# EI-CoreBioinformatics/portcullis

Measured on AMD Instinct MI355X. Metric: junc_reads_per_sec, higher is better.
Workload: dtype int32; 1 GPU; BASELINE configs[2]: synthetic 199999998 paired-end 150-bp reads, 25 contigs of GRCh38 lengths (3088286401 bp), 249999 junctions, orientation FR; reads_total=199999998, junctions_total=249999, contigs=25, reads_rank0=199999998, pairs_rank0=66692850

## Files before the change

### portcullis_amd/csrc/pjb_api.hip

```cpp
#include "pjb_host.hip.h"
#include "pjb_kernels.hip.h"
#include "pjb_chain.hip.h"
#include "pjb_flight.hip.h"

extern "C" {

namespace {
std::mutex g_host_mu;
std::map<void *, size_t> g_host_registered;
}
void *pjb_host_alloc(size_t bytes) {
    if (bytes >= ((size_t)8 << 20)) {
        const size_t huge = (size_t)2 << 20, len = (bytes + huge - 1) & ~(huge - 1);
        void *p = mmap(nullptr, len, PROT_READ | PROT_WRITE, MAP_PRIVATE | MAP_ANONYMOUS, -1, 0);
        if (p != MAP_FAILED) {
            (void)madvise(p, len, MADV_HUGEPAGE);
            const size_t nt = std::min<size_t>(4, len >> 24);
            auto touch = [&](size_t t) {
                const size_t per = ((len / std::max<size_t>(nt, 1)) + huge - 1) & ~(huge - 1), a = std::min(len, per * t), b = std::min(len, a + per);
                for (size_t o = a; o < b; o += 4096) ((volatile uint8_t *)p)[o] = 0;
            };
            if (nt <= 1) touch(0);
            else {
                std::vector<std::thread> th;
// ... 165 lines not shown
    release_pooled_slabs(c);
    if (c->rows_pinned) (void)hipHostFree(c->rows_pinned);
    if (c->rows_table) (void)dev_free(c, c->rows_table);
    bam_stage_clear(c);
    for (int k = 0; k < PJB_MAX_QUEUED; k++) {
        CtlSlot &S = c->sl[k];
        if (S.pub) (void)hipHostFree(S.pub);
        if (S.batches_pinned) (void)hipHostFree(S.batches_pinned);
        for (auto &ev : S.ev)
            if (ev) (void)hipEventDestroy(ev);
        if (S.ev_rows) (void)hipEventDestroy(S.ev_rows);
        if (S.ev_done) (void)hipEventDestroy(S.ev_done);
        Buf *sb[] = {&S.x_q, &S.x_spos, &S.x_send, &S.x_gapoff, &S.x_zlist, &S.x_scnt, &S.x_codes, &S.cstats, &S.err, &S.gencount, &S.batches, &S.rows, &S.tile_cnt, &S.tile_stats, &S.splidx, &S.splpoff, &S.splrec, &S.tile_soff, &S.chunk_tile, &S.scan_parts, &S.members, &S.okey, &S.g,
                     &S.rec, &S.jidbam, &S.jkey, &S.total, &S.bitmap, &S.wrank, &S.pagecnt, &S.pagerank, &S.ends, &S.firstid,
                     &S.key[0], &S.key[1], &S.idx[0], &S.idx[1], &S.hist, &S.hist_scan, &S.hist_part, &S.bintotal, &S.scan_tiles, &S.jid, &S.seg, &S.runfirst,
                     &S.runstart, &S.ent, &S.entsum, &S.frag, &S.fragj, &S.masks, &S.acc, &S.ancl, &S.ancr, &S.genlist, &S.runs};
        for (Buf *b : sb) release(c, *b);
        hipEvent_t evs[] = {S.ev_k1, S.ev_xk1, S.ev_fork, S.ev_join, S.ev_fork2, S.ev_join2};
        for (hipEvent_t e : evs)
            if (e) (void)hipEventDestroy(e);
        if (S.main) (void)hipStreamDestroy(S.main);
        if (S.side) (void)hipStreamDestroy(S.side);
    }
    if (c->mirror_hdr) (void)hipHostFree(c->mirror_hdr);
    for (int k = 0; k < 2; k++) {
        if (c->stage[k]) (void)hipHostFree(c->stage[k]);
        if (c->stage_ev[k]) (void)hipEventDestroy(c->stage_ev[k]);
    }
    Buf *all[] = {&c->b_cursor, &c->b_scan_tiles, &c->b_hasx, &c->b_xtotal, &c->b_fasta_raw, &c->b_inf_comp, &c->b_inf_out, &c->b_inf_blocks, &c->b_inf_status, &c->b_inf_scratch, &c->b_inf_bitmap,
                  &c->b_bam_seg, &c->b_bam_rec, &c->b_bam_ctl, &c->f_pos, &c->f_cigoff, &c->f_cigar, &c->f_codes,
                  &c->x_pos, &c->x_endx, &c->x_q, &c->x_prefq, &c->x_ce, &c->x_bound, &c->x_de, &c->x_dropped, &c->x_zlist, &c->x_cnt,
// ... 476 lines not shown
}

int pjb_set_option(pjb_ctx *c, const char *name, int64_t value) {
    if (!c || !name) return PJB_ERR_ARG;
    if (c->n_fl) return fail(c, PJB_ERR_STATE, "set_option: target %d is still queued", c->fl[0].tid);
    const std::string n = name;
    if (n == "overlap") c->side_stream = value != 0;
    else if (n == "dense_ids") c->dense_ids = value != 0;
    else if (n == "extra_dense") c->extra_dense_only = value != 0;
    else if (n == "sort_floor") c->sort_floor = (u32)std::max<int64_t>(1, std::min<int64_t>(value, 1 << 30));
    else if (n == "window_skip") c->window_skip = value != 0;
    else if (n == "run_sort") c->run_sort = value != 0;
    else if (n == "run_window") {
        if (value < 0 || value > (int64_t)RUN_W) return fail(c, PJB_ERR_ARG, "set_option: run_window takes 0 (the default, %u) to %u", RUN_W, RUN_W);
        c->run_window = (u32)value;
    } else if (n == "pair_range") {
        int shift = -1;
        for (int k = 0; k <= PAIR_RANGE_SHIFT_MAX; k++)
            if (value == (int64_t)1 << k) shift = k;
        if (shift < 0) return fail(c, PJB_ERR_ARG, "set_option: pair_range takes 1, 2, 4, 8, 16 or 32 slices a range (the default: %d)", 1 << PAIR_RANGE_SHIFT_DEFAULT);
        c->pair_range_shift = shift;
    } else if (n == "grow_batch") {
        if (value < 0 || value > 32768) return fail(c, PJB_ERR_ARG, "set_option: grow_batch takes 0 (the default: what the pool holds) to 32768 trees");
        c->model.grow_batch = (u32)value;
    } else if (n == "knn_chunk") {
        if (value < 0 || value > (1 << 22)) return fail(c, PJB_ERR_ARG, "set_option: knn_chunk takes 0 (the default: sized to fill the chip) to %d base rows", 1 << 22);
        c->model.knn_chunk = (u32)value;
    } else if (n == "mem_limit") {
        if (value < 0) return fail(c, PJB_ERR_ARG, "set_option: mem_limit takes 0 (the default: no limit) or a number of bytes");
        std::lock_guard<std::mutex> lk(c->mem.mu);
// ... 47 lines not shown
```

### portcullis_amd/csrc/pjb_chain.hip.h

```cpp
#pragma once

constexpr unsigned K6_BLOCKS = 128;

static size_t rows_upper_bound(const pjb_ctx *c) {
    size_t n = c->rows_n;
    for (int k = 0; k < c->n_fl; k++)
        if (c->fl[k].queued) n += c->fl[k].lim.junc_limit;
    return n;
}

static void wait_flight(pjb_ctx *c, Flight &f) {
    if (f.queued) (void)hipEventSynchronize(c->sl[f.slot].ev_done);
}

static int rows_table_reserve(pjb_ctx *c, Flight &f, u32 JL) {
    size_t old = rows_upper_bound(c);
    if (old + JL <= c->rows_cap) return PJB_OK;
    for (int k = 0; k < c->n_fl; k++)
        if (c->fl[k].queued && &c->fl[k] != &f) wait_flight(c, c->fl[k]);
    int rc = rows_sync(c);
    if (rc) return rc;
    old = std::min(old, c->rows_cap);
    const size_t ncap = std::max<size_t>((old + JL) * 3 / 2, 1024);
    pjb_junction_row *nd = (pjb_junction_row *)dev_alloc(c, MEM_ROWS, ncap * sizeof(pjb_junction_row));
// ... 2 lines not shown
        HIP_TRY(c, hipMemcpyAsync(nd, c->rows_table, old * sizeof(pjb_junction_row), hipMemcpyDeviceToDevice, c->stream4));
        HIP_TRY(c, hipStreamSynchronize(c->stream4));
    }
    if (c->rows_table) bury(c, c->rows_table);
    c->rows_table = nd;
    c->rows_cap = ncap;
    return PJB_OK;
}

struct Chain {
    pjb_ctx *c;
    Flight &f;
    CtlSlot &S;
    hipStream_t st, service;
    GroupTab GT;
    bool group, fast_codes, any_x, stage_events, xk1, dense_moved, entropy_forked;
    int n_members;
    int32_t ref_len;
    KeyFmt kf;
    u32 PL, JL, SL;
    u32 n_tiles, pair_blocks, range_blocks, slots_lim, n_slices_lim, gen_cap, pack_nn;
    int range_shift;
    size_t n_words;
    int64_t row_base, mirror_base;
    u32 rs_tiles, run_cap, ro_tiles, plan_tiles;
    bool run_route, first_hist_done;
    int sort_bits, n_pass, pass_bits[16], cur;
    RunOut ro;
    u64 *ro_total, *ro_key[2];
    u32 *run_dest, *ro_idx[2];
    u64 *d_err;
    ContigStats *d_cs;
    const u32 *d_P, *d_J, *d_slots;
    MemberStats *d_members;
    u32 *d_member_junc, *d_tile_lo, *d_gen_cnt;
    Pairs pr;
};

struct ChainScope {
    pjb_ctx *c;
    hipStream_t stream = c->stream;
    Buf *scan_tiles = c->scan_tiles;
    int pool = c->cur_pool;
    ~ChainScope() {
        c->stream = stream;
// ... 58 lines not shown
    ch.row_base = ahead ? -1 : (int64_t)c->rows_n;
    ch.mirror_base = ahead ? -1 : (int64_t)c->mirror_rows;
    ch.pair_blocks = std::max<u32>(1, (PL + 255) / 256);
    ch.gen_cap = lim.list_cap ? lim.list_cap : (c->list_cap_forced ? c->list_cap_forced : gen_list_cap(PL));
    ch.pack_nn = (u64)ch.n_tiles * K1_TILE < (1ull << 28) ? 1u : 0u;
    ch.range_shift = c->pair_range_shift;
    ch.slots_lim = frag_slots_limit(JL, PL, ch.range_shift);
    ch.range_blocks = std::max<u32>(1, (frag_ranges(PL, ch.range_shift) + 3) / 4);
    ch.n_slices_lim = (PL + 63) / 64 + 1;
    ch.n_words = ((size_t)std::max(ch.ref_len, 1) + 63) / 64;
    ch.stage_events = c->ktime && c->ktime_only.empty();
    ch.xk1 = c->extra && !c->extra_dense_only && !ch.group && !f.x_k1 && !f.x_pre;
    ch.rs_tiles = std::max<u32>(1, (PL + RS_TILE - 1) / RS_TILE);
    ch.run_route = lim.dense && lim.run_sort;
    ch.run_cap = (u32)std::min<u64>((u64)PL / 8 + 64ull * ch.rs_tiles, 0xfff00000ull);
    ch.ro_tiles = (ch.run_cap + RS_TILE - 1) / RS_TILE;
    if (ch.run_route) {
        ch.ro.cap = ch.run_cap;
        ch.ro.window = c->run_window ? std::min<u32>(c->run_window, RUN_W) : RUN_W;
        ch.ro.tile_bits = std::max(1, bits_of((uint64_t)ch.rs_tiles));
    }
    ch.sort_bits = lim.dense ? std::max(1, bits_of((uint64_t)ch.SL)) + (ch.run_route ? ch.ro.tile_bits : 0) : ch.kf.total_bits;
    ch.plan_tiles = ch.run_route ? ch.ro_tiles : ch.rs_tiles;
    ch.first_hist_done = lim.dense && !ch.run_route;
    ch.n_pass = std::max(1, (ch.sort_bits + c->radix_max_bits - 1) / c->radix_max_bits);
    for (int p = 0; p < ch.n_pass; p++) ch.pass_bits[p] = ch.sort_bits / ch.n_pass + (p < ch.sort_bits % ch.n_pass ? 1 : 0);
    return PJB_OK;
}

static RunOut run_carve(Chain &ch, int &rc) {
    pjb_ctx *c = ch.c;
    CtlSlot &S = ch.S;
    RunOut ro = ch.ro;
    auto al = [](size_t b) { return (b + 255) & ~(size_t)255; };
    const u32 rs_tiles = ch.rs_tiles, run_cap = ch.run_cap;
    const size_t slack = (size_t)run_cap + RS_TILE;
    const size_t at_tf = 256, at_tn = at_tf + al((size_t)rs_tiles * 4), at_key = at_tn + al((size_t)rs_tiles * 4), at_cnt = at_key + al(slack * 8),
                 at_dest = at_cnt + al((size_t)run_cap * 4), at_k0 = at_dest + al((size_t)run_cap * 4), at_k1 = at_k0 + al(slack * 8),
                 at_i0 = at_k1 + al(slack * 8), at_i1 = at_i0 + al(slack * 4), at_end = at_i1 + al(slack * 4);
    if ((rc = ensure(c, S.runs, at_end))) return ro;
    uint8_t *b = (uint8_t *)S.runs.p;
    ro.n_runs = (u32 *)b;
    ch.ro_total = (u64 *)(b + 8);
    ro.tile_first = (u32 *)(b + at_tf);
    ro.tile_n = (u32 *)(b + at_tn);
    ro.key = (u64 *)(b + at_key);
    ro.cnt = (u32 *)(b + at_cnt);
    ch.run_dest = (u32 *)(b + at_dest);
    ch.ro_key[0] = (u64 *)(b + at_k0);
    ch.ro_key[1] = (u64 *)(b + at_k1);
    ch.ro_idx[0] = (u32 *)(b + at_i0);
    ch.ro_idx[1] = (u32 *)(b + at_i1);
    return ro;
}

static int chain_room(Chain &ch) {
    pjb_ctx *c = ch.c;
    Flight &f = ch.f;
    CtlSlot &S = ch.S;
    const std::vector<DevBatch> &batches = f.batches;
    const u32 PL = ch.PL, JL = ch.JL, n_tiles = ch.n_tiles;
    const size_t n_words = ch.n_words, N = (size_t)f.n_reads;
    const u32 plan_tiles = ch.plan_tiles;
    const int dbits = ch.pass_bits[0];
    const bool dense = f.lim.dense;
    int rc;
    if (batches.size() + 2 > S.batches_pinned_cap) {
        if (S.batches_pinned) (void)hipHostFree(S.batches_pinned);
        S.batches_pinned = nullptr;
        S.batches_pinned_cap = 0;
        const size_t cap = std::max<size_t>(batches.size() * 2 + 2, 16);
        HIP_TRY(c, hipHostMalloc((void **)&S.batches_pinned, cap * sizeof(DevBatch), hipHostMallocDefault));
        S.batches_pinned_cap = cap;
    }
    memcpy(S.batches_pinned, batches.data(), batches.size() * sizeof(DevBatch));
    const struct { Buf *b; size_t bytes; bool whole; } once[] = {
        {&S.scan_parts, sizeof(ScanPart) * K1S_BLOCKS, false},
        {&c->b_cursor, sizeof(RowCursor), false},
// ... 36 lines not shown
        {&S.frag, (size_t)ch.slots_lim * F_WORDS * 4},
        {&S.fragj, (size_t)ch.slots_lim * 4},
        {&S.acc, (size_t)JL * F_WORDS * 4 + 16},
        {&S.ancl, (size_t)JL * 4 + 16},
        {&S.ancr, (size_t)JL * 4 + 16},
        {&S.jkey, (size_t)JL * 8 + 16},
        {&S.rows, (size_t)JL * sizeof(pjb_junction_row) + 16},
        {&S.entsum, (size_t)JL * 8 + 16},
        {&S.bitmap, n_words * 8 + 16, dense},
        {&S.wrank, n_words * 4 + 16, dense},
        {&S.pagecnt, ((n_words >> KD_PAGE_SHIFT) + 1) * 4 + 16, dense},
        {&S.pagerank, ((n_words >> KD_PAGE_SHIFT) + 1) * 4 + 16, dense},
        {&S.ends, (size_t)JL * DENSE_ENDS * 4 + 32, dense},
        {&S.firstid, (size_t)JL * 4 + 16, dense},
        {&S.masks, (size_t)ch.n_slices_lim * 8 * 2 + (size_t)ch.n_slices_lim * 4, dense},
        {&S.hist, (size_t)plan_tiles * (1u << dbits) * 4},
        {&S.hist_scan, (size_t)plan_tiles * (1u << dbits) * 4},
        {&S.bintotal, (size_t)4 << dbits},
        {&S.hist_part, (size_t)((plan_tiles + RSP_TILES - 1) / RSP_TILES) * (1u << dbits) * 4},
        {&S.x_q, N + 16, ch.xk1},
        {&S.x_spos, N * 4 + 16, ch.xk1},
        {&S.x_send, N * 4 + 16, ch.xk1},
        {&S.x_zlist, (size_t)X_ZCAP * 8, ch.xk1},
        {&S.x_scnt, X_SCNT_BYTES, ch.xk1},
    };
    for (const auto &r : room)
        if (r.on && (rc = ensure(c, *r.b, r.bytes))) return rc;
    ch.dense_moved = was[0] != S.bitmap.p || was[1] != S.ends.p || was[2] != S.pagecnt.p;
    if (ch.run_route) {
        ch.ro = run_carve(ch, rc);
        if (rc) return rc;
    }
    if ((rc = rows_table_reserve(c, f, JL))) return rc;
    if (!S.pub) {
        HIP_TRY(c, hipHostMalloc((void **)&S.pub, PUB_BYTES, hipHostMallocMapped | hipHostMallocPortable));
        void *dp = nullptr;
        if (hipHostGetDevicePointer(&dp, S.pub, 0) != hipSuccess || !dp) return fail(c, PJB_ERR_HIP, "hipHostGetDevicePointer(control block) failed");
        S.pub_dev = (uint8_t *)dp;
    }
    ch.d_members = (MemberStats *)S.members.p;
    ch.d_member_junc = (u32 *)(ch.d_members + GROUP_MAX);
    ch.d_tile_lo = ch.d_member_junc + GROUP_MAX;
    ch.d_err = (u64 *)S.err.p;
    ch.d_cs = (ContigStats *)S.cstats.p;
    ch.d_P = &ch.d_cs->P;
    ch.d_J = &ch.d_cs->J;
    ch.d_slots = &ch.d_cs->n_slots;
// ... 27 lines not shown
    }
    if (!S.at_rest) {
        HIP_TRY(c, hipMemsetAsync(S.err.p, 0xff, 8, st));
        HIP_TRY(c, hipMemsetAsync(S.gencount.p, 0, GEN_SHARDS * GEN_CNT_STRIDE * 4, st));
        HIP_TRY(c, hipMemsetAsync(ch.d_member_junc, 0, GROUP_MAX * 4, st));
    }
    S.at_rest = false;
    HIP_TRY(c, hipEventRecord(S.ev[0], st));
    if (f.lim.dense) {
        if (!S.dense_at_rest || ch.dense_moved) {
            HIP_TRY(c, hipMemsetAsync(S.bitmap.p, 0, S.bitmap.cap, st));
            HIP_TRY(c, hipMemsetAsync(S.pagecnt.p, 0, S.pagecnt.cap, st));
            HIP_TRY(c, hipMemsetAsync(S.ends.p, 0xff, S.ends.cap, st));
        }
        S.dense_at_rest = false;
    }
    f.pr = ch.pr;
    return PJB_OK;
}

static int chain_k1(Chain &ch) {
    pjb_ctx *c = ch.c;
    Flight &f = ch.f;
    CtlSlot &S = ch.S;
    const std::vector<DevBatch> &batches = f.batches;
    const hipStream_t st = ch.st;
    const GroupTab &GT = ch.GT;
    const KeyFmt kf = ch.kf;
    const u32 n_tiles = ch.n_tiles;
    const bool k1_late = getenv("PJB_K1_SERIAL_LATE") != nullptr;
// ... 91 lines not shown
        return rc;
    LAUNCH(c, "kd_table", kd_table, dim3(cand_blocks), dim3(256), (const u64 *)cand, (const u64 *)S.ent.p, (const u32 *)cand_rank, kf, JL,
           (const u32 *)S.ends.p, (const u32 *)S.firstid.p, (const u64 *)S.total.p, (u64 *)S.jkey.p, (int32_t *)S.ancl.p, (int32_t *)S.ancr.p, ch.d_cs,
           (const u32 *)ch.d_gen_cnt, ch.gen_cap, ch.SL, ch.ro.n_runs, ch.range_shift);
    LAUNCH(c, "kd_assign", kd_assign, dim3(ch.rs_tiles), dim3(256), okey, ch.d_P, kf, (const u64 *)S.bitmap.p, (const u32 *)S.wrank.p,
           (const u32 *)S.ends.p, (const u32 *)S.firstid.p, JL, (const u64 *)S.total.p, (u32 *)S.jidbam.p, (u32 *)S.acc.p, (const u64 *)S.jkey.p,
           (const int32_t *)S.ancl.p, (const int32_t *)S.ancr.p, ch.d_err, ch.d_cs, ch.run_route ? 0 : ch.pass_bits[0], (u32 *)S.hist.p, ch.ro);
    if ((rc = chain_fork(ch, S.ev_fork, S.ev_join, f.forked, chain_k4b))) return rc;
    LAUNCH(c, "kd_reset", kd_reset, dim3(cand_blocks), dim3(256), (const u64 *)cand, (const u32 *)cand_rank, kf, JL, (const ContigStats *)ch.d_cs,
           (u64 *)S.bitmap.p, (u32 *)S.ends.p, (u32 *)S.pagecnt.p);
    S.dense_at_rest = true;
    return PJB_OK;
}

static const char *const rs_names[4] = {"rs_hist", "rs_panel_sums", "rs_panel_scan", "rs_scatter"};
static const char *const ro_names[6] = {"ro_hist", "ro_panel_sums", "ro_panel_scan", "ro_scatter", "ro_offsets", "rs_place"};

template <typename K>
static int sort_pass(Chain &ch, const void *kin_v, void *kout_v, const u32 *vin, u32 *vout, int shift, int bits, const u32 *d_n, u32 tiles,
                     const char *const *names) {
    pjb_ctx *c = ch.c;
    CtlSlot &S = ch.S;
    const K *kin = (const K *)kin_v;
    K *kout = (K *)kout_v;
    if (!(shift == 0 && ch.first_hist_done))
        LAUNCH(c, names[0], rs_hist<K>, dim3(tiles), dim3(256), kin, d_n, shift, bits, (u32 *)S.hist.p, tiles);
    {
        const u32 nb = 1u << bits, n_panels = (tiles + RSP_TILES - 1) / RSP_TILES;
        LAUNCH(c, names[1], rs_panel_sums, dim3(n_panels, (nb + 255) / 256), dim3(256), (const u32 *)S.hist.p, tiles, nb, (u32 *)S.hist_part.p);
        LAUNCH(c, names[2], rs_panel_scan, dim3(n_panels, (nb + 255) / 256), dim3(256), (const u32 *)S.hist.p, (const u32 *)S.hist_part.p, tiles, nb,
               (u32 *)S.hist_scan.p, (u32 *)S.bintotal.p);
// ... 5 lines not shown
    case 9: RS_SCATTER(9); break;
    case 10: RS_SCATTER(10); break;
    case 11: RS_SCATTER(11); break;
    default: RS_SCATTER(0); break;
    }
#undef RS_SCATTER
    return PJB_OK;
}

static int chain_sort(Chain &ch) {
    pjb_ctx *c = ch.c;
    Flight &f = ch.f;
    CtlSlot &S = ch.S;
    const RunOut &ro = ch.ro;
    int rc = PJB_OK, cur = 0, shift = 0;
    for (int p = 0; p < ch.n_pass; p++) {
        const int bits = ch.pass_bits[p];
        if (bits <= 0) break;
        if (ch.run_route) {
            rc = sort_pass<u64>(ch, p == 0 ? (const void *)ro.key : (const void *)ch.ro_key[cur], ch.ro_key[cur ^ 1], p == 0 ? nullptr : (const u32 *)ch.ro_idx[cur],
                                ch.ro_idx[cur ^ 1], shift, bits, (const u32 *)ro.n_runs, ch.ro_tiles, ro_names);
        } else {
            const u32 *vin = p == 0 ? nullptr : (const u32 *)S.idx[cur].p;
            u32 *vout = (u32 *)S.idx[cur ^ 1].p;
            if (f.lim.dense) rc = sort_pass<u32>(ch, p == 0 ? S.jidbam.p : S.key[cur].p, S.key[cur ^ 1].p, vin, vout, shift, bits, ch.d_P, ch.rs_tiles, rs_names);
            else rc = sort_pass<u64>(ch, p == 0 ? S.okey.p : S.key[cur].p, S.key[cur ^ 1].p, vin, vout, shift, bits, ch.d_P, ch.rs_tiles, rs_names);
        }
        if (rc) return rc;
        cur ^= 1;
        shift += bits;
    }
    f.n_pass = ch.n_pass;
    if (ch.run_route) {
        const u32 *order = ch.ro_idx[cur];
        if ((rc = run_scan(c, ro_names[4], RunCountFn{(const u32 *)ro.cnt, order}, RunDestSink{ch.run_dest, order}, (u64)ch.run_cap, ch.ro_total, (const u32 *)ro.n_runs)))
            return rc;
        cur = 1;
        LAUNCH(c, ro_names[5], rs_place, dim3(ch.rs_tiles), dim3(256), (const u32 *)S.jidbam.p, ch.d_P, (const u64 *)ro.key, (const u32 *)ch.run_dest,
               (const u32 *)ro.tile_first, (const u32 *)ro.tile_n, ch.run_cap, ro.tile_bits, (u32 *)S.key[cur].p, (u32 *)S.idx[cur].p);
        f.n_pass = 1;
    }
    ch.cur = cur;
    f.sidx = (const u32 *)S.idx[cur].p;
    f.jid_sorted = f.lim.dense ? (const u32 *)S.key[cur].p : (const u32 *)S.jid.p;
    STAGE_EVENT(2);
    return PJB_OK;
}

static int chain_entropy(Chain &ch) {
    pjb_ctx *c = ch.c;
    CtlSlot &S = ch.S;
    LAUNCH(c, "k5_entropy_sum", k5_entropy_sum, dim3(std::max<u32>(1, (ch.JL + 15) / 16)), dim3(256), (const u32 *)S.seg.p, (const u32 *)S.runfirst.p,
           (const u32 *)S.runstart.p, ch.d_J, (double *)S.entsum.p);
// ... 145 lines not shown
```

### portcullis_amd/csrc/pjb_device.hip.h

```cpp
#pragma once

#include <hip/hip_runtime.h>
#include <stdint.h>

#include "../../include/portcullis_amd.h"

namespace pjb {

typedef unsigned long long u64;
typedef unsigned int u32;

struct DevBatch {
    const int32_t *pos;
    const uint16_t *flag;
    const uint8_t *mapq;
    const uint8_t *xs;
    const int32_t *l_qseq;
    const int32_t *mtid;
    const int32_t *mpos;
    const uint32_t *cig_off;
    const uint32_t *cigar;
    const uint32_t *seq_off;
    const uint8_t *seq4;
    const u64 *name_hash;
// ... 623 lines not shown
        rem &= ~m;
    }
    if ((rem >> lane) & 1ull) atomicAdd(&h[d], 1u);
}

constexpr u32 RUN_W = 2048;
struct RunOut {
    u64 *key;
    u32 *cnt;
    u32 *tile_first;
    u32 *tile_n;
    u32 *n_runs;
    u32 cap;
    u32 window;
    int tile_bits;
};

enum {
    F_N = 0, F_R1P, F_R1N, F_R2P, F_R2N, F_MS, F_XSP, F_XSN, F_UM, F_BPP, F_PPP, F_REL, F_DIST,
    F_MAXMINANC, F_UP, F_DOWN, F_MAXMMES, F_MAXMINMATCH,
    F_FIRSTMIS,
    F_PAD19,
    F_MISM_LO, F_MISM_HI,
    F_JAD0,
    F_WORDS = 48
};
__device__ __forceinline__ void acc_rest_state(u32 *acc, u64 n_junc) {
    const u64 n = n_junc * F_WORDS, step = (u64)gridDim.x * blockDim.x;
    for (u64 t = (u64)blockIdx.x * blockDim.x + threadIdx.x; t < n; t += step) acc[t] = (t % F_WORDS) == F_FIRSTMIS ? 100000000u : 0u;
}

// ... 2 lines not shown
```

### portcullis_amd/csrc/pjb_host.hip.h

```cpp
#pragma once
#include "pjb_device.hip.h"
#include "pjb_extra_types.hip.h"
#include "pjb_memory.hip.h"

#include <algorithm>
#include <sys/mman.h>
#include <thread>
#include <chrono>
#include <cstdarg>
#include <cstdio>
#include <cstdlib>
#include <cstring>
#include <map>
#include <memory>
#include <mutex>
#include <string>
#include <thread>
#include <unordered_map>
#include <vector>

using namespace pjb;


inline thread_local std::string g_create_error;
// ... 69 lines not shown
    bool run_sort = false;
};

struct CtlSlot {
    Buf cstats, err, gencount, batches, rows;
    Buf x_q, x_spos, x_send, x_gapoff, x_zlist, x_scnt, x_codes;
    Buf tile_cnt, tile_stats, splidx, splpoff, splrec, tile_soff, chunk_tile;
    Buf scan_parts;
    u32 scan_epoch = 0;
    Buf members;
    Buf okey, rec, g, jidbam;
    hipEvent_t ev_k1 = nullptr;
    hipEvent_t ev_xk1 = nullptr;
    Buf total, bitmap, wrank, ends, firstid, key[2], idx[2], hist, hist_scan, hist_part, bintotal, scan_tiles;
    Buf runs;
    Buf pagecnt, pagerank;
    Buf jid, seg, runfirst, runstart, ent, entsum, frag, fragj, acc, ancl, ancr, jkey, genlist, masks;
    bool dense_at_rest = false;
    hipStream_t main = nullptr, side = nullptr;
    hipEvent_t ev_fork = nullptr, ev_join = nullptr, ev_fork2 = nullptr, ev_join2 = nullptr;
    uint8_t *pub = nullptr, *pub_dev = nullptr;
    DevBatch *batches_pinned = nullptr;
    size_t batches_pinned_cap = 0;
    bool at_rest = false;
    hipEvent_t ev[PJB_N_STAGES + 2] = {};
    hipEvent_t ev_rows = nullptr, ev_done = nullptr;
};
struct EvPool {
    std::vector<hipEvent_t> ev;
    size_t used = 0;
// ... 129 lines not shown
    std::vector<void *> graveyard;
    std::mutex grave_mu;
    size_t last_rows_n = 0;
    uint8_t *mirror = nullptr;
    size_t mirror_cap = 0;
    int64_t *mirror_hdr = nullptr;
    size_t mirror_rows = 0;
    int64_t mirror_acc[5] = {0, 0, 0, INT32_MAX, 0};
    pjb_timing timing;
    int radix_max_bits = 11;
    double junc_per_read = 0;
    u32 sort_floor = 1u << 16;
    bool window_skip = true;
    bool run_sort = true;
    u32 run_window = 0;
    int pair_range_shift = PAIR_RANGE_SHIFT_DEFAULT;
    u32 list_cap_forced = 0;
    bool k1_serial = true;
    hipEvent_t last_k1_ev = nullptr;
    int k1s_blocks_forced = 0;
    bool ktime = false;
    std::vector<std::string> knames;
    std::vector<int64_t> kcount;
    std::vector<double> kms;
    std::vector<std::string> ktime_only;
    Buf *scan_tiles = nullptr;
    Buf b_scan_tiles;
    Buf b_inf_comp, b_inf_out, b_inf_blocks, b_inf_status, b_inf_scratch, b_inf_bitmap;
    Buf b_dfl_in, b_dfl_sym, b_dfl_slots, b_dfl_size, b_dfl_off, b_dfl_packed;
    Buf b_bam_seg, b_bam_rec, b_bam_ctl;
// ... 559 lines not shown
```

### portcullis_amd/csrc/pjb_k2_sort.hip.h

```cpp
#pragma once

#include "pjb_device.hip.h"

namespace pjb {


template <typename K>
__global__ __launch_bounds__(256) void rs_hist(const K *keys, const u32 *np, int shift, int bits, u32 *hist, u32 n_tiles) {
    __shared__ u32 h[RS_MAX_BINS];
    const u32 n = *np;
    const u32 nb = 1u << bits;
    for (u32 d = threadIdx.x; d < nb; d += 256) h[d] = 0;
    __syncthreads();
    const u32 base = blockIdx.x * RS_TILE;
    const u32 mask = nb - 1;
    K kk[RS_ITEMS];
#pragma unroll
    for (int k = 0; k < RS_ITEMS; k++) {
        const u32 i = base + k * 256 + threadIdx.x;
        kk[k] = i < n ? keys[i] : (K)0;
    }
#pragma unroll
    for (int k = 0; k < RS_ITEMS; k++) {
        const u32 i = base + k * 256 + threadIdx.x;
// ... 175 lines not shown
    }
    __syncthreads();
#pragma unroll
    for (int r = 0; r < RS_ITEMS; r++) {
        const u32 i = base + r * 64 + lane;
        if (i < n) ibuf[(rkp[r >> 1] >> ((r & 1) * 16)) & 0xffffu] = val[r];
    }
    __syncthreads();
#pragma unroll
    for (int r = 0; r < RS_ITEMS; r++) {
        const u32 j = r * 256 + threadIdx.x;
        if (j < cnt) vout[delta[(digp[r >> 1] >> ((r & 1) * 16)) & 0xffffu] + j] = ibuf[j];
    }
}

struct RunCountFn {
    const u32 *cnt, *order;
    __device__ u64 operator()(u64 i) const { return cnt[order[i]]; }
};
struct RunDestSink {
    u32 *dest;
    const u32 *order;
    __device__ void operator()(u64 i, u64, u64 ex) const { dest[order[i]] = (u32)ex; }
};
__global__ __launch_bounds__(256) void rs_place(const u32 *jid_bam, const u32 *np, const u64 *run_key, const u32 *run_dest, const u32 *tile_first,
                                                const u32 *tile_n, u32 run_cap, int tile_bits, u32 *kout, u32 *vout) {
    __shared__ u32 s_dest[RUN_W];
    __shared__ unsigned short s_wcnt[4][RUN_W];
    const u32 n = *np;
    const u32 tile = blockIdx.x;
    if ((u64)tile * RS_TILE >= n) return;
    for (u32 d = threadIdx.x; d < 2 * RUN_W; d += 256) ((u32 *)&s_wcnt[0][0])[d] = 0;
    const u32 tf = tile_first[tile], tn = tf < run_cap ? min(tile_n[tile], min(RUN_W, run_cap - tf)) : 0u;
    for (u32 e = threadIdx.x; e < tn; e += 256) s_dest[(u32)(run_key[tf + e] >> tile_bits) & (RUN_W - 1u)] = run_dest[tf + e];
    const int w = __builtin_amdgcn_readfirstlane(threadIdx.x >> 6), lane = lane_id();
    unsigned short *wc = s_wcnt[w];
    const u32 base = tile * RS_TILE + w * (RS_TILE / 4);
    const u64 lt = (1ull << lane) - 1;
    u32 id[RS_ITEMS];
// ... 43 lines not shown
```

### portcullis_amd/csrc/pjb_k2d_ids.hip.h

```cpp
#pragma once

#include "pjb_device.hip.h"

namespace pjb {

constexpr int DENSE_ENDS = 8;
constexpr u32 DENSE_EMPTY = 0xffffffffu;

__device__ __forceinline__ u32 start_rank(const u64 *bitmap, const u32 *wrank, int32_t start) {
    const u32 w = (u32)start >> 6;
    return wrank[w] + (u32)__popcll(bitmap[w] & ((1ull << (start & 63)) - 1ull));
}
struct PopcFn {
    const u64 *words;
    __device__ u64 operator()(u64 i) const { return (u64)__popcll(words[i]); }
};
__global__ __launch_bounds__(256) void kd_ends(const u64 *cand, KeyFmt kf, const u64 *bitmap, const u32 *wrank, u32 junc_limit, u32 *ends,
                                               u32 *cand_rank, ContigStats *cs) {
    const u32 n = cs->n_cand;
    for (u32 p = blockIdx.x * 256 + threadIdx.x; p < n; p += gridDim.x * 256) {
        int32_t s, e;
        unpack_key(kf, cand[p], s, e);
        const u32 rs = start_rank(bitmap, wrank, s);
        cand_rank[p] = rs;
// ... 100 lines not shown
            unpack_key(kf, k, s, e);
            id = first_id[rs] + ends_below(ends, rs, (u32)e);
            valid = id < junc_limit;
            if (valid) jkey[id] = k;
        }
        if (valid) {
            const int32_t lo = (int32_t)(u32)a, hi = (int32_t)(u32)(a >> 32);
            if (lo < __hip_atomic_load(&anc_l[id], __ATOMIC_RELAXED, __HIP_MEMORY_SCOPE_AGENT)) atomicMin(&anc_l[id], lo);
            if (hi > __hip_atomic_load(&anc_r[id], __ATOMIC_RELAXED, __HIP_MEMORY_SCOPE_AGENT)) atomicMax(&anc_r[id], hi);
        }
    }
}

constexpr int KDA_PER = 4;
static_assert(RUN_W == 256 * 8, "kd_assign compacts eight table entries a thread");
__device__ __forceinline__ void runs_close_chain(ContigStats *cs) {
    atomicOr(&cs->overflow, OVF_RUNS);
    cs->P = 0;
    cs->J = 0;
    cs->n_slots = 0;
    cs->n_slices = 0;
}
__global__ __launch_bounds__(256) void kd_assign(const u64 *key, const u32 *np, KeyFmt kf, const u64 *bitmap, const u32 *wrank, const u32 *ends,
                                                 const u32 *first_id, u32 junc_limit, const u64 *total, u32 *jid_bam, u32 *acc, const u64 *jkey,
                                                 const int32_t *anc_l, const int32_t *anc_r, u64 *err, ContigStats *cs_chk, int hist_bits, u32 *hist,
                                                 RunOut ro) {
    __shared__ u32 s_h[4096];
    __shared__ u32 s_run[4];
    __shared__ u32 s_rscan[4];
    const u32 n = *np;
    if (n == 0) {
        if (hist_bits > 0)
            for (u32 d = threadIdx.x; d < (1u << hist_bits); d += 256) hist[(size_t)blockIdx.x * (1u << hist_bits) + d] = 0;
        return;
    }
    {
        const u64 J = *total;
// ... 122 lines not shown
                atomicSub(ro.n_runs, tot);
                b = 0xffffffffu;
                runs_close_chain(cs_chk);
            }
            s_run[2] = b;
            ro.tile_first[blockIdx.x] = b == 0xffffffffu ? 0u : b;
            ro.tile_n[blockIdx.x] = b == 0xffffffffu ? 0u : tot;
        }
        __syncthreads();
        const u32 first = s_run[2];
        if (first == 0xffffffffu) return;
        at += first;
#pragma unroll
        for (int k = 0; k < 8; k++)
            if (c[k]) {
                ro.key[at] = ((u64)(lo + threadIdx.x * 8u + (u32)k) << ro.tile_bits) | (u64)blockIdx.x;
                ro.cnt[at] = c[k];
                at++;
            }
    }
}

}
```

Before: 31.48 billion reads/s.

## Replace radix sort of run keys with per-id slab bucketing and wave walk

Run placement used to sort the (id, tile) run keys with multi-pass radix sort before a count scan. Now kd_assign also accumulates, per junction id, the total count and the min and max tile using atomics. A scan over ids sizes a slab of tile slots per id, rr_fill drops each run into its slot, and rr_walk does a wave-level prefix over each id's slab to compute run destinations, resetting the per-id state as it goes. This removes the radix sort passes and their histogram buffers. In exchange it adds atomics in kd_assign, extra per-id buffers and memsets, and an overflow fallback when the slab's room is exceeded.

```diff
diff --git a/portcullis_amd/csrc/pjb_api.hip b/portcullis_amd/csrc/pjb_api.hip
--- a/portcullis_amd/csrc/pjb_api.hip
+++ b/portcullis_amd/csrc/pjb_api.hip
@@ -203,7 +203,7 @@
         Buf *sb[] = {&S.x_q, &S.x_spos, &S.x_send, &S.x_gapoff, &S.x_zlist, &S.x_scnt, &S.x_codes, &S.cstats, &S.err, &S.gencount, &S.batches, &S.rows, &S.tile_cnt, &S.tile_stats, &S.splidx, &S.splpoff, &S.splrec, &S.tile_soff, &S.chunk_tile, &S.scan_parts, &S.members, &S.okey, &S.g,
                      &S.rec, &S.jidbam, &S.jkey, &S.total, &S.bitmap, &S.wrank, &S.pagecnt, &S.pagerank, &S.ends, &S.firstid,
                      &S.key[0], &S.key[1], &S.idx[0], &S.idx[1], &S.hist, &S.hist_scan, &S.hist_part, &S.bintotal, &S.scan_tiles, &S.jid, &S.seg, &S.runfirst,
-                     &S.runstart, &S.ent, &S.entsum, &S.frag, &S.fragj, &S.masks, &S.acc, &S.ancl, &S.ancr, &S.genlist, &S.runs};
+                     &S.runstart, &S.ent, &S.entsum, &S.frag, &S.fragj, &S.masks, &S.acc, &S.ancl, &S.ancr, &S.genlist, &S.runs, &S.id_total, &S.id_t0, &S.id_t1, &S.slab};
         for (Buf *b : sb) release(c, *b);
         hipEvent_t evs[] = {S.ev_k1, S.ev_xk1, S.ev_fork, S.ev_join, S.ev_fork2, S.ev_join2};
         for (hipEvent_t e : evs)
@@ -710,6 +710,9 @@
     else if (n == "run_window") {
         if (value < 0 || value > (int64_t)RUN_W) return fail(c, PJB_ERR_ARG, "set_option: run_window takes 0 (the default, %u) to %u", RUN_W, RUN_W);
         c->run_window = (u32)value;
+    } else if (n == "run_slab") {
+        if (value < 0 || value > 0xfff00000ll) return fail(c, PJB_ERR_ARG, "set_option: run_slab takes 0 (the default: the run list's room) or the slab's entries");
+        c->run_slab = (u32)value;
     } else if (n == "pair_range") {
         int shift = -1;
         for (int k = 0; k <= PAIR_RANGE_SHIFT_MAX; k++)
diff --git a/portcullis_amd/csrc/pjb_chain.hip.h b/portcullis_amd/csrc/pjb_chain.hip.h
--- a/portcullis_amd/csrc/pjb_chain.hip.h
+++ b/portcullis_amd/csrc/pjb_chain.hip.h
@@ -40,7 +40,7 @@
     CtlSlot &S;
     hipStream_t st, service;
     GroupTab GT;
-    bool group, fast_codes, any_x, stage_events, xk1, dense_moved, entropy_forked;
+    bool group, fast_codes, any_x, stage_events, xk1, dense_moved, runs_moved, entropy_forked;
     int n_members;
     int32_t ref_len;
     KeyFmt kf;
@@ -49,12 +49,13 @@
     int range_shift;
     size_t n_words;
     int64_t row_base, mirror_base;
-    u32 rs_tiles, run_cap, ro_tiles, plan_tiles;
+    u32 rs_tiles, run_cap;
     bool run_route, first_hist_done;
     int sort_bits, n_pass, pass_bits[16], cur;
     RunOut ro;
-    u64 *ro_total, *ro_key[2];
-    u32 *run_dest, *ro_idx[2];
+    RunSlab slab;
+    u64 *ro_total;
+    u32 *run_dest;
     u64 *d_err;
     ContigStats *d_cs;
     const u32 *d_P, *d_J, *d_slots;
@@ -143,31 +144,36 @@
     ch.rs_tiles = std::max<u32>(1, (PL + RS_TILE - 1) / RS_TILE);
     ch.run_route = lim.dense && lim.run_sort;
     ch.run_cap = (u32)std::min<u64>((u64)PL / 8 + 64ull * ch.rs_tiles, 0xfff00000ull);
-    ch.ro_tiles = (ch.run_cap + RS_TILE - 1) / RS_TILE;
     if (ch.run_route) {
         ch.ro.cap = ch.run_cap;
         ch.ro.window = c->run_window ? std::min<u32>(c->run_window, RUN_W) : RUN_W;
         ch.ro.tile_bits = std::max(1, bits_of((uint64_t)ch.rs_tiles));
-    }
-    ch.sort_bits = lim.dense ? std::max(1, bits_of((uint64_t)ch.SL)) + (ch.run_route ? ch.ro.tile_bits : 0) : ch.kf.total_bits;
-    ch.plan_tiles = ch.run_route ? ch.ro_tiles : ch.rs_tiles;
+        ch.slab.room = c->run_slab ? c->run_slab : run_slab_room(ch.run_cap);
+        ch.slab.junc_limit = JL;
+    }
+    ch.sort_bits = lim.dense ? std::max(1, bits_of((uint64_t)ch.SL)) : ch.kf.total_bits;
     ch.first_hist_done = lim.dense && !ch.run_route;
     ch.n_pass = std::max(1, (ch.sort_bits + c->radix_max_bits - 1) / c->radix_max_bits);
     for (int p = 0; p < ch.n_pass; p++) ch.pass_bits[p] = ch.sort_bits / ch.n_pass + (p < ch.sort_bits % ch.n_pass ? 1 : 0);
     return PJB_OK;
 }
 
-static RunOut run_carve(Chain &ch, int &rc) {
-    pjb_ctx *c = ch.c;
-    CtlSlot &S = ch.S;
-    RunOut ro = ch.ro;
+static int run_carve(Chain &ch) {
+    pjb_ctx *c = ch.c;
+    CtlSlot &S = ch.S;
+    RunOut &ro = ch.ro;
+    RunSlab &sl = ch.slab;
     auto al = [](size_t b) { return (b + 255) & ~(size_t)255; };
-    const u32 rs_tiles = ch.rs_tiles, run_cap = ch.run_cap;
-    const size_t slack = (size_t)run_cap + RS_TILE;
-    const size_t at_tf = 256, at_tn = at_tf + al((size_t)rs_tiles * 4), at_key = at_tn + al((size_t)rs_tiles * 4), at_cnt = at_key + al(slack * 8),
-                 at_dest = at_cnt + al((size_t)run_cap * 4), at_k0 = at_dest + al((size_t)run_cap * 4), at_k1 = at_k0 + al(slack * 8),
-                 at_i0 = at_k1 + al(slack * 8), at_i1 = at_i0 + al(slack * 4), at_end = at_i1 + al(slack * 4);
-    if ((rc = ensure(c, S.runs, at_end))) return ro;
+    const u32 rs_tiles = ch.rs_tiles, run_cap = ch.run_cap, JL = ch.JL;
+    const size_t at_tf = 256, at_tn = at_tf + al((size_t)rs_tiles * 4), at_key = at_tn + al((size_t)rs_tiles * 4), at_cnt = at_key + al((size_t)run_cap * 8),
+                 at_dest = at_cnt + al((size_t)run_cap * 4), at_base = at_dest + al((size_t)run_cap * 4), at_off = at_base + al((size_t)JL * 4),
+                 at_end = at_off + al((size_t)JL * 4);
+    const void *was[4] = {S.id_total.p, S.id_t0.p, S.id_t1.p, S.slab.p};
+    int rc;
+    if ((rc = ensure(c, S.runs, at_end)) || (rc = ensure(c, S.id_total, (size_t)JL * 4 + 16)) || (rc = ensure(c, S.id_t0, (size_t)JL * 4 + 16)) ||
+        (rc = ensure(c, S.id_t1, (size_t)JL * 4 + 16)) || (rc = ensure(c, S.slab, (size_t)sl.room * 4 + 16)))
+        return rc;
+    ch.runs_moved = was[0] != S.id_total.p || was[1] != S.id_t0.p || was[2] != S.id_t1.p || was[3] != S.slab.p;
     uint8_t *b = (uint8_t *)S.runs.p;
     ro.n_runs = (u32 *)b;
     ch.ro_total = (u64 *)(b + 8);
@@ -176,11 +182,15 @@
     ro.key = (u64 *)(b + at_key);
     ro.cnt = (u32 *)(b + at_cnt);
     ch.run_dest = (u32 *)(b + at_dest);
-    ch.ro_key[0] = (u64 *)(b + at_k0);
-    ch.ro_key[1] = (u64 *)(b + at_k1);
-    ch.ro_idx[0] = (u32 *)(b + at_i0);
-    ch.ro_idx[1] = (u32 *)(b + at_i1);
-    return ro;
+    ro.id_total = (u32 *)S.id_total.p;
+    ro.id_t0 = (u32 *)S.id_t0.p;
+    ro.id_t1 = (u32 *)S.id_t1.p;
+    sl.id_base = (u32 *)(b + at_base);
+    sl.slab_off = (u32 *)(b + at_off);
+    sl.slab = (u32 *)S.slab.p;
+    sl.grand = ch.ro_total;
+    sl.n_ids = (const u64 *)S.total.p;
+    return PJB_OK;
 }
 
 static int chain_room(Chain &ch) {
@@ -190,7 +200,8 @@
     const std::vector<DevBatch> &batches = f.batches;
     const u32 PL = ch.PL, JL = ch.JL, n_tiles = ch.n_tiles;
     const size_t n_words = ch.n_words, N = (size_t)f.n_reads;
-    const u32 plan_tiles = ch.plan_tiles;
+    const u32 plan_tiles = ch.rs_tiles;
+    const bool passes = !ch.run_route;
     const int dbits = ch.pass_bits[0];
     const bool dense = f.lim.dense;
     int rc;
@@ -257,10 +268,10 @@
         {&S.ends, (size_t)JL * DENSE_ENDS * 4 + 32, dense},
         {&S.firstid, (size_t)JL * 4 + 16, dense},
         {&S.masks, (size_t)ch.n_slices_lim * 8 * 2 + (size_t)ch.n_slices_lim * 4, dense},
-        {&S.hist, (size_t)plan_tiles * (1u << dbits) * 4},
-        {&S.hist_scan, (size_t)plan_tiles * (1u << dbits) * 4},
-        {&S.bintotal, (size_t)4 << dbits},
-        {&S.hist_part, (size_t)((plan_tiles + RSP_TILES - 1) / RSP_TILES) * (1u << dbits) * 4},
+        {&S.hist, (size_t)plan_tiles * (1u << dbits) * 4, passes},
+        {&S.hist_scan, (size_t)plan_tiles * (1u << dbits) * 4, passes},
+        {&S.bintotal, (size_t)4 << dbits, passes},
+        {&S.hist_part, (size_t)((plan_tiles + RSP_TILES - 1) / RSP_TILES) * (1u << dbits) * 4, passes},
         {&S.x_q, N + 16, ch.xk1},
         {&S.x_spos, N * 4 + 16, ch.xk1},
         {&S.x_send, N * 4 + 16, ch.xk1},
@@ -270,10 +281,7 @@
     for (const auto &r : room)
         if (r.on && (rc = ensure(c, *r.b, r.bytes))) return rc;
     ch.dense_moved = was[0] != S.bitmap.p || was[1] != S.ends.p || was[2] != S.pagecnt.p;
-    if (ch.run_route) {
-        ch.ro = run_carve(ch, rc);
-        if (rc) return rc;
-    }
+    if (ch.run_route && (rc = run_carve(ch))) return rc;
     if ((rc = rows_table_reserve(c, f, JL))) return rc;
     if (!S.pub) {
         HIP_TRY(c, hipHostMalloc((void **)&S.pub, PUB_BYTES, hipHostMallocMapped | hipHostMallocPortable));
@@ -331,6 +339,15 @@
             HIP_TRY(c, hipMemsetAsync(S.ends.p, 0xff, S.ends.cap, st));
         }
         S.dense_at_rest = false;
+    }
+    if (ch.run_route) {
+        if (!S.runs_at_rest || ch.runs_moved) {
+            HIP_TRY(c, hipMemsetAsync(S.id_total.p, 0, S.id_total.cap, st));
+            HIP_TRY(c, hipMemsetAsync(S.id_t0.p, 0xff, S.id_t0.cap, st));
+            HIP_TRY(c, hipMemsetAsync(S.id_t1.p, 0, S.id_t1.cap, st));
+            HIP_TRY(c, hipMemsetAsync(S.slab.p, 0, S.slab.cap, st));
+        }
+        S.runs_at_rest = false;
     }
     f.pr = ch.pr;
     return PJB_OK;
@@ -452,7 +469,8 @@
 }
 
 static const char *const rs_names[4] = {"rs_hist", "rs_panel_sums", "rs_panel_scan", "rs_scatter"};
-static const char *const ro_names[6] = {"ro_hist", "ro_panel_sums", "ro_panel_scan", "ro_scatter", "ro_offsets", "rs_place"};
+static const char *const rr_names[4] = {"rr_scan", "rr_fill", "rr_walk", "rs_place"};
+constexpr unsigned RR_BLOCKS = 64;
 
 template <typename K>
 static int sort_pass(Chain &ch, const void *kin_v, void *kout_v, const u32 *vin, u32 *vout, int shift, int bits, const u32 *d_n, u32 tiles,
@@ -488,29 +506,27 @@
     CtlSlot &S = ch.S;
     const RunOut &ro = ch.ro;
     int rc = PJB_OK, cur = 0, shift = 0;
-    for (int p = 0; p < ch.n_pass; p++) {
+    for (int p = 0; p < ch.n_pass && !ch.run_route; p++) {
         const int bits = ch.pass_bits[p];
         if (bits <= 0) break;
-        if (ch.run_route) {
-            rc = sort_pass<u64>(ch, p == 0 ? (const void *)ro.key : (const void *)ch.ro_key[cur], ch.ro_key[cur ^ 1], p == 0 ? nullptr : (const u32 *)ch.ro_idx[cur],
-                                ch.ro_idx[cur ^ 1], shift, bits, (const u32 *)ro.n_runs, ch.ro_tiles, ro_names);
-        } else {
-            const u32 *vin = p == 0 ? nullptr : (const u32 *)S.idx[cur].p;
-            u32 *vout = (u32 *)S.idx[cur ^ 1].p;
-            if (f.lim.dense) rc = sort_pass<u32>(ch, p == 0 ? S.jidbam.p : S.key[cur].p, S.key[cur ^ 1].p, vin, vout, shift, bits, ch.d_P, ch.rs_tiles, rs_names);
-            else rc = sort_pass<u64>(ch, p == 0 ? S.okey.p : S.key[cur].p, S.key[cur ^ 1].p, vin, vout, shift, bits, ch.d_P, ch.rs_tiles, rs_names);
-        }
+        const u32 *vin = p == 0 ? nullptr : (const u32 *)S.idx[cur].p;
+        u32 *vout = (u32 *)S.idx[cur ^ 1].p;
+        if (f.lim.dense) rc = sort_pass<u32>(ch, p == 0 ? S.jidbam.p : S.key[cur].p, S.key[cur ^ 1].p, vin, vout, shift, bits, ch.d_P, ch.rs_tiles, rs_names);
+        else rc = sort_pass<u64>(ch, p == 0 ? S.okey.p : S.key[cur].p, S.key[cur ^ 1].p, vin, vout, shift, bits, ch.d_P, ch.rs_tiles, rs_names);
         if (rc) return rc;
         cur ^= 1;
         shift += bits;
     }
     f.n_pass = ch.n_pass;
     if (ch.run_route) {
-        const u32 *order = ch.ro_idx[cur];
-        if ((rc = run_scan(c, ro_names[4], RunCountFn{(const u32 *)ro.cnt, order}, RunDestSink{ch.run_dest, order}, (u64)ch.run_cap, ch.ro_total, (const u32 *)ro.n_runs)))
+        if ((rc = run_scan(c, rr_names[0], SlabTermFn{(const u32 *)ro.id_total, (const u32 *)ro.id_t0, (const u32 *)ro.id_t1}, SlabOffSink{ch.slab.id_base, ch.slab.slab_off},
+                           (u64)ch.SL, ch.ro_total, (const u32 *)S.total.p)))
             return rc;
+        LAUNCH(c, rr_names[1], rr_fill, dim3(RR_BLOCKS), dim3(256), ro, ch.slab, ch.d_cs);
+        LAUNCH(c, rr_names[2], rr_walk, dim3(RR_BLOCKS), dim3(RR_WALK_T), ro, ch.slab, ch.run_dest, (const ContigStats *)ch.d_cs);
+        S.runs_at_rest = true;
         cur = 1;
-        LAUNCH(c, ro_names[5], rs_place, dim3(ch.rs_tiles), dim3(256), (const u32 *)S.jidbam.p, ch.d_P, (const u64 *)ro.key, (const u32 *)ch.run_dest,
+        LAUNCH(c, rr_names[3], rs_place, dim3(ch.rs_tiles), dim3(256), (const u32 *)S.jidbam.p, ch.d_P, (const u64 *)ro.key, (const u32 *)ch.run_dest,
                (const u32 *)ro.tile_first, (const u32 *)ro.tile_n, ch.run_cap, ro.tile_bits, (u32 *)S.key[cur].p, (u32 *)S.idx[cur].p);
         f.n_pass = 1;
     }
diff --git a/portcullis_amd/csrc/pjb_device.hip.h b/portcullis_amd/csrc/pjb_device.hip.h
--- a/portcullis_amd/csrc/pjb_device.hip.h
+++ b/portcullis_amd/csrc/pjb_device.hip.h
@@ -661,7 +661,30 @@
     u32 cap;
     u32 window;
     int tile_bits;
-};
+    u32 *id_total;
+    u32 *id_t0;
+    u32 *id_t1;
+};
+
+__device__ __forceinline__ void runs_close_chain(ContigStats *cs) {
+    atomicOr(&cs->overflow, OVF_RUNS);
+    cs->P = 0;
+    cs->J = 0;
+    cs->n_slots = 0;
+    cs->n_slices = 0;
+}
+
+constexpr u32 RUN_SLAB_MULT = 1;
+__host__ __device__ inline u32 run_slab_room(u32 run_cap) {
+    const u64 r = (u64)run_cap * RUN_SLAB_MULT;
+    return (u32)(r < 0xfff00000ull ? r : 0xfff00000ull);
+}
+__host__ __device__ inline u32 run_slab_span(u32 total, u32 t0, u32 t1) { return total != 0u && t0 <= t1 ? t1 - t0 + 1u : 0u; }
+__host__ __device__ inline u64 run_slab_term(u32 total, u32 t0, u32 t1) { return ((u64)total << 32) | (u64)run_slab_span(total, t0, t1); }
+__host__ __device__ inline u32 run_slab_base(u64 exclusive) { return (u32)(exclusive >> 32); }
+__host__ __device__ inline u32 run_slab_off(u64 exclusive) { return (u32)exclusive; }
+__host__ __device__ inline u64 run_slab_at(u32 off, u32 t0, u32 tile) { return (u64)off + (u64)(tile - t0); }
+__host__ __device__ inline bool run_slab_fits(u64 grand, u32 n_pairs, u32 room) { return (u32)(grand >> 32) == n_pairs && (u32)grand <= room; }
 
 enum {
     F_N = 0, F_R1P, F_R1N, F_R2P, F_R2N, F_MS, F_XSP, F_XSN, F_UM, F_BPP, F_PPP, F_REL, F_DIST,
diff --git a/portcullis_amd/csrc/pjb_host.hip.h b/portcullis_amd/csrc/pjb_host.hip.h
--- a/portcullis_amd/csrc/pjb_host.hip.h
+++ b/portcullis_amd/csrc/pjb_host.hip.h
@@ -107,6 +107,8 @@
     hipEvent_t ev_xk1 = nullptr;
     Buf total, bitmap, wrank, ends, firstid, key[2], idx[2], hist, hist_scan, hist_part, bintotal, scan_tiles;
     Buf runs;
+    Buf id_total, id_t0, id_t1, slab;
+    bool runs_at_rest = false;
     Buf pagecnt, pagerank;
     Buf jid, seg, runfirst, runstart, ent, entsum, frag, fragj, acc, ancl, ancr, jkey, genlist, masks;
     bool dense_at_rest = false;
@@ -266,6 +268,7 @@
     bool window_skip = true;
     bool run_sort = true;
     u32 run_window = 0;
+    u32 run_slab = 0;
     int pair_range_shift = PAIR_RANGE_SHIFT_DEFAULT;
     u32 list_cap_forced = 0;
     bool k1_serial = true;
diff --git a/portcullis_amd/csrc/pjb_k2_sort.hip.h b/portcullis_amd/csrc/pjb_k2_sort.hip.h
--- a/portcullis_amd/csrc/pjb_k2_sort.hip.h
+++ b/portcullis_amd/csrc/pjb_k2_sort.hip.h
@@ -213,15 +213,113 @@
     }
 }
 
-struct RunCountFn {
-    const u32 *cnt, *order;
-    __device__ u64 operator()(u64 i) const { return cnt[order[i]]; }
+struct SlabTermFn {
+    const u32 *id_total, *id_t0, *id_t1;
+    __device__ u64 operator()(u64 i) const { return run_slab_term(id_total[i], id_t0[i], id_t1[i]); }
 };
-struct RunDestSink {
-    u32 *dest;
-    const u32 *order;
-    __device__ void operator()(u64 i, u64, u64 ex) const { dest[order[i]] = (u32)ex; }
+struct SlabOffSink {
+    u32 *id_base, *slab_off;
+    __device__ void operator()(u64 i, u64, u64 ex) const {
+        id_base[i] = run_slab_base(ex);
+        slab_off[i] = run_slab_off(ex);
+    }
 };
+struct RunSlab {
+    u32 *id_base;
+    u32 *slab_off;
+    u32 *slab;
+    const u64 *grand;
+    const u64 *n_ids;
+    u32 room, junc_limit;
+};
+__global__ __launch_bounds__(256) void rr_fill(RunOut ro, RunSlab sl, ContigStats *cs) {
+    const u32 n_pairs = cs->P;
+    if (n_pairs == 0) return;
+    if (!run_slab_fits(*sl.grand, n_pairs, sl.room)) {
+        if (blockIdx.x == 0 && threadIdx.x == 0) runs_close_chain(cs);
+        return;
+    }
+    const u32 nr = *ro.n_runs, n = nr < ro.cap ? nr : ro.cap;
+    const u64 tile_mask = (1ull << ro.tile_bits) - 1ull;
+    for (u32 i = blockIdx.x * 256 + threadIdx.x; i < n; i += gridDim.x * 256) {
+        const u64 k = ro.key[i];
+        const u32 id = (u32)(k >> ro.tile_bits), tile = (u32)(k & tile_mask);
+        if (id >= sl.junc_limit) continue;
+        const u64 at = run_slab_at(sl.slab_off[id], ro.id_t0[id], tile);
+        if (at < (u64)sl.room) sl.slab[at] = i + 1u;
+    }
+}
+constexpr int RR_W = 8;
+constexpr int RR_WALK_T = 512;
+__global__ __launch_bounds__(RR_WALK_T) void rr_walk(RunOut ro, RunSlab sl, u32 *run_dest, const ContigStats *cs) {
+    const u64 nj = *sl.n_ids;
+    const u32 n_ids = (u32)(nj < (u64)sl.junc_limit ? nj : (u64)sl.junc_limit);
+    const bool closed = cs->P == 0;
+    const int lane = lane_id();
+    const u32 wave = blockIdx.x * (u32)(RR_WALK_T / 64) + (threadIdx.x >> 6), n_waves = gridDim.x * (u32)(RR_WALK_T / 64);
+    for (u64 i0 = (u64)wave * 64; i0 < n_ids; i0 += (u64)n_waves * 64) {
+        const u64 id = i0 + (u64)lane;
+        u32 tot = 0u, t0 = 0xffffffffu, t1 = 0u;
+        if (id < n_ids) {
+            tot = ro.id_total[id];
+            t0 = ro.id_t0[id];
+            t1 = ro.id_t1[id];
+            if (tot != 0u || t0 != 0xffffffffu || t1 != 0u) {
+                ro.id_total[id] = 0u;
+                ro.id_t0[id] = 0xffffffffu;
+                ro.id_t1[id] = 0u;
+            }
+        }
+        if (closed) continue;
+        const u32 span = run_slab_span(tot, t0, t1);
+        u32 base = 0u, off = 0u;
+        if (span) {
+            base = sl.id_base[id];
+            off = sl.slab_off[id];
+        }
+        for (u64 todo = __ballot(span > (u32)RR_W); todo; todo &= todo - 1) {
+            const int src = __ffsll((long long)todo) - 1;
+            const u32 sp = (u32)__builtin_amdgcn_readlane((int)span, src), so = (u32)__builtin_amdgcn_readlane((int)off, src);
+            u32 sum = (u32)__builtin_amdgcn_readlane((int)base, src);
+            for (u32 e0 = 0; e0 < sp; e0 += 64) {
+                const u64 at = (u64)so + e0 + (u32)lane;
+                const bool in = e0 + (u32)lane < sp && at < (u64)sl.room;
+                const u32 v = in ? sl.slab[at] : 0u;
+                const bool run = v != 0u && v <= ro.cap;
+                const u32 c = run ? ro.cnt[v - 1u] : 0u;
+                const u32 inc = wave_iscan(c);
+                if (run) run_dest[v - 1u] = sum + inc - c;
+                if (v) sl.slab[at] = 0u;
+                sum += (u32)__builtin_amdgcn_readlane((int)inc, 63);
+            }
+        }
+        const int g = lane / RR_W, sub = lane % RR_W;
+        u64 at[RR_W];
+        u32 sb[RR_W], v[RR_W], c[RR_W];
+#pragma unroll
+        for (int k = 0; k < RR_W; k++) {
+            const int src = g + k * (64 / RR_W);
+            const u32 sp = (u32)__shfl((int)span, src, 64), so = (u32)__shfl((int)off, src, 64);
+            sb[k] = (u32)__shfl((int)base, src, 64);
+            at[k] = (u64)so + (u32)sub;
+            const bool in = sp <= (u32)RR_W && (u32)sub < sp && at[k] < (u64)sl.room;
+            v[k] = in ? sl.slab[at[k]] : 0u;
+        }
+#pragma unroll
+        for (int k = 0; k < RR_W; k++) c[k] = v[k] != 0u && v[k] <= ro.cap ? ro.cnt[v[k] - 1u] : 0u;
+#pragma unroll
+        for (int k = 0; k < RR_W; k++) {
+            u32 inc = c[k];
+#pragma unroll
+            for (int o = 1; o < RR_W; o <<= 1) {
+                const u32 t = (u32)__shfl_up((int)inc, o, RR_W);
+                if (sub >= o) inc += t;
+            }
+            if (v[k] != 0u && v[k] <= ro.cap) run_dest[v[k] - 1u] = sb[k] + inc - c[k];
+            if (v[k]) sl.slab[at[k]] = 0u;
+        }
+    }
+}
 __global__ __launch_bounds__(256) void rs_place(const u32 *jid_bam, const u32 *np, const u64 *run_key, const u32 *run_dest, const u32 *tile_first,
                                                 const u32 *tile_n, u32 run_cap, int tile_bits, u32 *kout, u32 *vout) {
     __shared__ u32 s_dest[RUN_W];
diff --git a/portcullis_amd/csrc/pjb_k2d_ids.hip.h b/portcullis_amd/csrc/pjb_k2d_ids.hip.h
--- a/portcullis_amd/csrc/pjb_k2d_ids.hip.h
+++ b/portcullis_amd/csrc/pjb_k2d_ids.hip.h
@@ -138,13 +138,6 @@
 
 constexpr int KDA_PER = 4;
 static_assert(RUN_W == 256 * 8, "kd_assign compacts eight table entries a thread");
-__device__ __forceinline__ void runs_close_chain(ContigStats *cs) {
-    atomicOr(&cs->overflow, OVF_RUNS);
-    cs->P = 0;
-    cs->J = 0;
-    cs->n_slots = 0;
-    cs->n_slices = 0;
-}
 __global__ __launch_bounds__(256) void kd_assign(const u64 *key, const u32 *np, KeyFmt kf, const u64 *bitmap, const u32 *wrank, const u32 *ends,
                                                  const u32 *first_id, u32 junc_limit, const u64 *total, u32 *jid_bam, u32 *acc, const u64 *jkey,
                                                  const int32_t *anc_l, const int32_t *anc_r, u64 *err, ContigStats *cs_chk, int hist_bits, u32 *hist,
@@ -297,9 +290,15 @@
 #pragma unroll
         for (int k = 0; k < 8; k++)
             if (c[k]) {
-                ro.key[at] = ((u64)(lo + threadIdx.x * 8u + (u32)k) << ro.tile_bits) | (u64)blockIdx.x;
+                const u32 id = lo + threadIdx.x * 8u + (u32)k;
+                ro.key[at] = ((u64)id << ro.tile_bits) | (u64)blockIdx.x;
                 ro.cnt[at] = c[k];
                 at++;
+                if (id < junc_limit) {
+                    atomicAdd(&ro.id_total[id], c[k]);
+                    atomicMin(&ro.id_t0[id], blockIdx.x);
+                    atomicMax(&ro.id_t1[id], blockIdx.x);
+                }
             }
     }
 }
```

Result: no change. 31.48 billion reads/s (median of 2 runs) (-0.0%).
